# hobincar/reconstruction-network-for-video-captioning

Measured on AMD Instinct MI355X. Metric: captions/sec (train step) MSVD bs=100 28x1536 feats, higher is better.
Workload: dtype bf16; 1 GPU; decoder + global reconstructor train step (fwd+bwd+clip+Adam), B=100 per GPU, F=28, D=R=1536, V=4188, E=468, H=512, A=128, T=31, dropout 0.5, LSTM cells; global_batch=100, parallelism=dp1, hipgraph=True, deferred_reconstructor_update=True, grad_allreduce=False

## Files before the change

reconstruction-network-for-video-captioning_amd/csrc/abi_step.inc:

```

int recnet_set_deferred_reconstructor_update(recnet_handle* h, int32_t on, void* stream) {
  REQUIRE_WS(h);
  FLUSH_PENDING(h, stream);
  h->defer_rec = on ? (on == 2 ? 2 : 1) : 0;
  LAUNCH_OK();
  return RECNET_OK;
}
int recnet_flush(recnet_handle* h, void* stream) {
  REQUIRE_WS(h);
  int r = flush_pending(h, (hipStream_t)stream, 1); if (r) return r;
  LAUNCH_OK();
  return RECNET_OK;
}
int recnet_set_dp_overlap(recnet_handle* h, int32_t on) {
  if (!h) return fail(RECNET_EINVAL, "null handle");
  h->ss.dp_overlap = on ? 1 : 0;
  return RECNET_OK;
}
int recnet_join_side(recnet_handle* h, void* stream) {
  REQUIRE_WS(h);
  if (h->ss.side_open && h->s2) { hipEventRecord(h->ev[EV_REC_DW_JOIN], h->s2); hipStreamWaitEvent((hipStream_t)stream, h->ev[EV_REC_DW_JOIN], 0); }
  h->ss.side_open = 0;
  LAUNCH_OK();
  return RECNET_OK;
}
int recnet_abort_step(recnet_handle* h) {
  if (!h) return fail(RECNET_EINVAL, "null handle");
  sched_reset(h);
  return RECNET_OK;
}
int recnet_mark_pending(recnet_handle* h) {
  if (!h) return fail(RECNET_EINVAL, "null handle");
  if (h->defer_rec) { h->maybe_pending = 1; h->images_maybe_stale = 1; }
  return RECNET_OK;
}

int recnet_forward_decoder(recnet_handle* h, const float* enc, const int64_t* targets, int32_t T,
                           const float* step_weight, int32_t train, uint32_t seed, float* hiddens_out,
                           recnet_scalars* scalars, void* stream) {
  REQUIRE_WS(h);
  if (!h->dec_bound) return fail(RECNET_ESTATE, "decoder not bound");
  if (!enc || !targets || !step_weight) return fail(RECNET_EINVAL, "null argument");
  if (check_T(h, T)) return fail(RECNET_EINVAL, "T out of range");
  hipStream_t st = (hipStream_t)stream;
  hipLaunchKernelGGL(set_u32_kernel, dim3(1), dim3(1), 0, st, h->ctrl, seed);
  int r = fwd_decoder(h, enc, targets, T, step_weight, train, hiddens_out, st); if (r) return r;
  if (scalars) hipLaunchKernelGGL(export_scalars_kernel, dim3(1), dim3(1), 0, st, h->scal, scalars);
  LAUNCH_OK();
  return RECNET_OK;
}

int recnet_forward_decoder_free(recnet_handle* h, const float* enc, const int64_t* targets, int32_t T,
                                const float* step_weight, int32_t train, uint32_t seed, float* hiddens_out,
                                int64_t* output_indices, recnet_scalars* scalars, void* stream) {
  REQUIRE_WS(h);
  if (!h->dec_bound) return fail(RECNET_ESTATE, "decoder not bound");
// ... 29 lines not shown
  return RECNET_OK;
}

int recnet_backward_reconstructor(recnet_handle* h, const float* enc, float grad_scale, float* dhiddens_out, void* stream) {
  REQUIRE_WS(h);
  FLUSH_PENDING(h, stream);
  h->ss.prezeroed = 0;
  if (!h->fwd_rec_done) return fail(RECNET_ESTATE, "backward_reconstructor before forward_reconstructor");
  if (!h->rG.out_weight) return fail(RECNET_ESTATE, "reconstructor gradients not bound");
  hipStream_t st = (hipStream_t)stream;
  float* dh = dhiddens_out ? dhiddens_out : h->dHsrec;
  int r = bwd_rec(h, grad_scale, dh, st);
  if (r) return r;
  if (dhiddens_out) copyf(dhiddens_out, h->dHsrec, (size_t)h->T_last * h->B * h->H, st);
  h->rec_bwd_done = 1;
  (void)enc;
  LAUNCH_OK();
  return RECNET_OK;
}

int recnet_backward_decoder(recnet_handle* h, const float* enc, const int64_t* targets, const float* dhiddens,
                            float grad_scale, void* stream) {
  REQUIRE_WS(h);
  h->ss.prezeroed = 0;
  if (!h->fwd_dec_done) return fail(RECNET_ESTATE, "backward_decoder before forward_decoder");
  if (!h->dGd.out_weight) return fail(RECNET_ESTATE, "decoder gradients not bound");
  if (!enc || !targets) return fail(RECNET_EINVAL, "null argument");
  int r = bwd_decoder(h, enc, targets, dhiddens, grad_scale, (hipStream_t)stream); if (r) return r;
  h->fwd_dec_done = 0;
  LAUNCH_OK();
  return RECNET_OK;
}

int recnet_add_reg_grad(recnet_handle* h, int32_t which, float grad_scale, void* stream) {
  REQUIRE_WS(h);
  FLUSH_PENDING(h, stream);
  if (which < 0 || which > 1 || !h->og[which].bound) return fail(RECNET_EINVAL, "model not bound");
  OptGroup& o = h->og[which];
  const float lam = which == 0 ? h->c.decoder_lambda_reg : h->c.reconstructor_lambda_reg;
  hipLaunchKernelGGL(add_reg_grad_kernel, dim3(o.nchunks), dim3(256), 0, (hipStream_t)stream, o.d_tab, o.d_chunks, o.d_pnorm, lam * grad_scale);
  LAUNCH_OK();
  return RECNET_OK;
}

int recnet_clip_grad_norm(recnet_handle* h, int32_t which, float max_norm, float* total_norm_out, void* stream) {
  REQUIRE_WS(h);
// ... 50 lines not shown
  const bool rec = h->kind != RECNET_REC_NONE && !h->ss.defer_now;
  hipStream_t sd = h->s2;
  hipStream_t sn = h->ss.hoist_par ? sd : st;
  h->ss.hoist_pending = 0;
  if (sn != st) { if (h->ss.hoist_fork_recorded) hipStreamWaitEvent(sd, h->ev[EV_HOIST_FORK], 0); else fork_to(h, EV_HOIST_FORK, st, sd); }
  if (sn != st && h->persist_dec) wait_chain(h, 0, sn);
  param_norms(h, 0, h->scal + RN_SCAL_DEC_REG, sn);
  if (rec) { param_norms(h, 1, h->scal + RN_SCAL_REC_REG, sn); gate_bias(h->rP.rnn_bias_ih_l0, h->rP.rnn_bias_hh_l0, h->bsum_r, h->R, h->rgru, sn); }
  if (split_upd) gate_bias(h->rP.rnn_bias_ih_l0, h->rP.rnn_bias_hh_l0, h->bsum_r, h->R, h->rgru, sn);
  {
    ZeroList z; z.cnt = 0;
    auto add = [&](float* p, size_t n) { if (p && n) { z.p[z.cnt] = p; z.n[z.cnt] = n; ++z.cnt; } };
    add(h->dGd.embedding_weight, (size_t)h->V * h->E); add(h->dGd.out_bias, h->V); add(h->bsum4, (size_t)4 * h->H);
    add(h->dGd.attn_b, h->A); add(h->dGd.attn_w_weight, h->A);
    if (rec || split_upd) { add(h->rG.out_bias, h->R); add(h->bsum4r, (size_t)4 * h->R); }
    hipLaunchKernelGGL(zero_list_kernel, dim3(512), dim3(256), 0, sn, z);
    h->ss.prezeroed = 1;
  }
  if (h->kind == RECNET_REC_GLOBAL) {
    hipLaunchKernelGGL(mean_over_f_kernel, dim3(ew_blocks((size_t)h->B * h->D)), dim3(256), 0, sn, h->ss.hoist_enc, h->B, h->F, h->D, h->encmean);
    h->ss.encmean_hoisted = 1;
  }
  if (sn != st) hipEventRecord(h->ev[EV_HOIST_DONE], sd);
}

static void side_after_decoder_fwd(recnet_handle* h, hipStream_t st) {
  hipStream_t sd = h->overlap ? h->s2 : st;
  const bool par = sd != st;
  h->ss.side_pending = 0;
  if (par) {
    if (h->ss.side_fork_recorded) {
      hipStreamWaitEvent(sd, h->ev[EV_SIDE_FORK], 0);
      if (h->kind == RECNET_REC_GLOBAL && h->persist_rec) wait_chain(h, 2, sd);
    } else fork_to(h, EV_SIDE_FORK, st, sd);
    h->ss.side_fork_recorded = 0; h->ss.gws_cur = h->gws2;
  }
  h->ss.join_pending = par; h->ss.join_recorded = 0; h->ss.side_tail_open = 0;
  if (par && h->kind != RECNET_REC_NONE) h->ss.gg_slots = 2 * (h->ncu > 192 ? h->ncu - 192 : 32);
  int r = dec_fwd_loss(h, h->ss.side_targets, h->ss.side_T, h->ss.side_stepw, 1, sd);
  if (!r) r = dec_bwd_out(h, 1.0f, sd);
  h->ss.gg_slots = 0;
  if (!r && par && h->ss.side_phase != 2) { dec_ctx_rows(h, h->ss.side_enc, 0, h->ss.side_T, sd); h->ss.ctx_done = 1; }
  if (h->ss.side_tail_open) hipEventRecord(h->ev[EV_SIDE_TAIL], sd);
  h->ss.gws_cur = h->gws;
  h->ss.side_err = r;
}

static int fwd_bwd_impl(recnet_handle* h, const float* enc, const int64_t* targets, int T, const float* stepw, hipStream_t st,
                        int phase, int early_opt) {
  const bool rec = h->kind != RECNET_REC_NONE;
  hipStream_t sd = h->overlap ? h->s2 : st;
  const bool par = sd != st;
  int r;
  bool s3_join = false;
  const float* dh = rec ? h->dHsrec : nullptr;
  h->ss.early_opt_done = 0;
  if (phase != 2) h->free_fwd = 0;
  if (phase != 2) h->ss.ctx_done = 0;
  const bool defer_static = h->defer_rec && (h->kind == RECNET_REC_GLOBAL || (h->defer_rec == 2 && h->kind == RECNET_REC_LOCAL)) && phase == 0 && early_opt >= 0 && par && h->s3 &&
                            (h->defer_rec != 2 || h->split_ok);
  const bool defer = defer_static && (h->defer_rec != 2 || T >= 2);
  if (!defer && h->defer_rec && phase != 2) {
    if (defer_static) { const int fr = flush_pending(h, st, 1); if (fr) return fr; }
    else if (h->maybe_pending) { const int fr = flush_pending(h, st, 0); if (fr) return fr; }
  }
  h->ss.defer_now = defer ? 1 : 0;
  h->ss.img_defer_now = (!defer_static && h->defer_rec && rec && h->lp && phase == 0 && early_opt >= 0 && par && h->s3 &&
                      (h->persist_rec_bwd || h->persist_loc_bwd || h->persist_big_bwd || (h->persist_loc && h->lc_steps))) ? 1 : 0;
  if (defer) h->defer_flags = early_opt;
  if (phase != 2) {
    h->ss.hoist_pending = 1; h->ss.hoist_enc = enc; h->ss.hoist_par = par ? 1 : 0;
    h->ss.norms_hoisted = 1;
    r = dec_fwd_chain(h, enc, targets, T, 1, st);
    if (h->ss.hoist_pending) hoist_side_work(h, st);
    if (!r && h->ss.defer_err) { r = h->ss.defer_err; h->ss.defer_err = 0; }
    if (r) { h->ss.norms_hoisted = 0; return r; }
    h->ss.side_targets = targets; h->ss.side_stepw = stepw; h->ss.side_enc = enc; h->ss.side_T = T; h->ss.side_phase = phase; h->ss.side_err = 0;
    h->ss.side_pending = 1;
    if (!(par && h->kind == RECNET_REC_GLOBAL)) side_after_decoder_fwd(h, st);
// ... 52 lines not shown
    }
    h->ss.gws_cur = h->gws;
    if (r) { h->ss.defer_now = 0; return r; }
    if (h->kind == RECNET_REC_GLOBAL && T < h->Tm)
      hipMemsetAsync(at_off(h, h->dGr, (size_t)T * h->B * h->ld4R), 0, (size_t)(h->Tm - T) * h->B * h->ld4R * (h->lp ? 2 : 4), sd);
    hipLaunchKernelGGL(set_u32_kernel, dim3(1), dim3(1), 0, sd, h->ctrl + RN_CTRL_PENDING, 1u);
    h->maybe_pending = 1; h->ss.early_opt_done = 1; h->ss.deferred_done = 1;
  }
  if (phase == 0 && rec && !h->ss.deferred_done) {
    if (par) h->ss.gws_cur = h->gws2;
    if (par && h->persist_dec_bwd) wait_chain(h, 1, sd);
    r = bwd_rec_deferred(h, sd, 0); if (r) return r;
    h->ss.gws_cur = h->gws;
    if (early_opt >= 0 && par) {
      const int f_s3 = h->R >= 2560 ? 1 : 0;
      hipStream_t so = (f_s3 && h->s3) ? h->s3 : sd;
      if (so != sd) fork_to(h, EV_OPT_FORK, sd, so);
      r = optimizer_step(h, early_opt, so, 1); if (r) return r;
      h->ss.early_opt_done = 1;
      s3_join = so != sd;
    }
  }
  h->ss.deferred_done = 0;
  r = dec_bwd_chain(h, dh, st); if (r) return r;
  if (par) fork_to(h, EV_DEC_DW_FORK, st, sd);
  r = dec_bwd_deferred(h, enc, targets, st, par ? sd : nullptr, (par && h->s3 && !s3_join) ? h->s3 : nullptr);
  h->ss.ctx_done = 0;
  if (r) return r;
  if (par) join_from(h, EV_TAIL_JOIN, st, sd);
  if (s3_join) { if (h->ss.in_fused) h->ss.s3_late = 1; else join_from(h, EV_S3_JOIN, st, h->s3); }
  h->fwd_dec_done = 0;
  h->ss.prezeroed = 0;
  return RECNET_OK;
}

static int fwd_bwd(recnet_handle* h, const float* enc, const int64_t* targets, int T, const float* stepw, hipStream_t st,
                   int phase = 0, int early_opt = -1) {
  const int r = fwd_bwd_impl(h, enc, targets, T, stepw, st, phase, early_opt);
  if (!r && phase != 1 && early_opt < 0 && h->og[0].bound && h->og[0].tab[0].g)
    hipLaunchKernelGGL(poison_mark_kernel, dim3(1), dim3(1), 0, st, h->og[0].tab[0].g, (const float*)(h->scal + RN_SCAL_POISON));
  h->ss.defer_now = 0;
  if (r) sched_reset(h);
  return r;
}

static int check_step_args(recnet_handle* h, const float* enc, const int64_t* targets, int T, const float* step_weight) {
// ... 7 lines not shown
int recnet_train_step_fwd_bwd(recnet_handle* h, const float* enc, const int64_t* targets, int32_t T,
                              const float* step_weight, uint32_t seed, recnet_scalars* scalars, void* stream) {
  REQUIRE_WS(h);
  FLUSH_PENDING(h, stream);
  { const int cr = check_step_args(h, enc, targets, T, step_weight); if (cr) return cr; }
  hipStream_t st = (hipStream_t)stream;
  hipLaunchKernelGGL(set_u32_kernel, dim3(1), dim3(1), 0, st, h->ctrl, seed);
  int r = fwd_bwd(h, enc, targets, T, step_weight, st); if (r) return r;
  if (scalars) hipLaunchKernelGGL(export_scalars_kernel, dim3(1), dim3(1), 0, st, h->scal, scalars);
  h->fwd_dec_done = 0;
  LAUNCH_OK();
  return RECNET_OK;
}

static void step_fail_cleanup(recnet_handle* h, hipStream_t st) {
  if (h->ss.s3_late && h->s3) join_from(h, EV_S3_JOIN, st, h->s3);
  recnet_abort_step(h);
  if (h->defer_rec) { h->maybe_pending = 1; h->images_maybe_stale = 1; }
}

static int fused_step(recnet_handle* h, const float* enc, const int64_t* targets, int T, const float* step_weight, int flags,
                      recnet_scalars* scalars, hipStream_t st) {
  h->ss.in_fused = 1;
  int r = fwd_bwd(h, enc, targets, T, step_weight, st, 0, flags); if (r) { h->ss.in_fused = 0; return r; }
  r = optimizer_step(h, flags, st, h->ss.early_opt_done ? 0 : -1); h->ss.in_fused = 0;
  if (r) { step_fail_cleanup(h, st); return r; }
  if (h->ss.s3_late) { join_from(h, EV_S3_JOIN, st, h->s3); h->ss.s3_late = 0; }
  h->ss.img_defer_now = 0;
  if (scalars) hipLaunchKernelGGL(export_scalars_kernel, dim3(1), dim3(1), 0, st, h->scal, scalars);
  h->fwd_dec_done = 0;
  LAUNCH_OK();
  return RECNET_OK;
}

int recnet_train_step(recnet_handle* h, const float* enc, const int64_t* targets, int32_t T,
                      const float* step_weight, uint32_t seed, int32_t step, recnet_scalars* scalars, void* stream) {
  REQUIRE_WS(h);
  if (!h->defer_rec) { const int fr_ = flush_pending(h, (hipStream_t)stream); if (fr_) return fr_; }
  int r = check_step_args(h, enc, targets, T, step_weight); if (r) return r;
  if (step < 1) return fail(RECNET_EINVAL, "step must be >= 1");
  hipStream_t st = (hipStream_t)stream;
  hipLaunchKernelGGL(set_u32_kernel, dim3(1), dim3(1), 0, st, h->ctrl, seed);
  hipLaunchKernelGGL(set_step_kernel, dim3(1), dim3(1), 0, st, (int32_t*)(h->ctrl + RN_CTRL_STEP), step);
  return fused_step(h, enc, targets, T, step_weight, RECNET_OPT_REG | RECNET_OPT_CLIP, scalars, st);
}

int recnet_train_step_dev(recnet_handle* h, const float* enc, const int64_t* targets, int32_t T, const float* step_weight,
                          uint32_t seed_base, int32_t flags, recnet_scalars* scalars, void* stream) {
  REQUIRE_WS(h);
  if (!h->defer_rec) { const int fr_ = flush_pending(h, (hipStream_t)stream); if (fr_) return fr_; }
  int r = check_step_args(h, enc, targets, T, step_weight); if (r) return r;
  hipStream_t st = (hipStream_t)stream;
  hipLaunchKernelGGL(advance_step_kernel, dim3(1), dim3(1), 0, st, (int32_t*)(h->ctrl + RN_CTRL_STEP), h->ctrl, seed_base);
  return fused_step(h, enc, targets, T, step_weight, flags, scalars, st);
}

int recnet_set_step(recnet_handle* h, int32_t step, void* stream) {
  REQUIRE_WS(h);
  hipLaunchKernelGGL(set_u32_kernel, dim3(1), dim3(1), 0, (hipStream_t)stream, h->ctrl + RN_CTRL_STEP, (uint32_t)step);
  LAUNCH_OK();
  return RECNET_OK;
}

int recnet_train_step_fwd_bwd_dev(recnet_handle* h, const float* enc, const int64_t* targets, int32_t T,
                                  const float* step_weight, uint32_t seed_base, recnet_scalars* scalars, void* stream) {
  REQUIRE_WS(h);
  FLUSH_PENDING(h, stream);
  { const int cr = check_step_args(h, enc, targets, T, step_weight); if (cr) return cr; }
  hipStream_t st = (hipStream_t)stream;
  hipLaunchKernelGGL(advance_step_kernel, dim3(1), dim3(1), 0, st, (int32_t*)(h->ctrl + RN_CTRL_STEP), h->ctrl, seed_base);
  int r = fwd_bwd(h, enc, targets, T, step_weight, st); if (r) return r;
  if (scalars) hipLaunchKernelGGL(export_scalars_kernel, dim3(1), dim3(1), 0, st, h->scal, scalars);
  h->fwd_dec_done = 0;
// ... 32 lines not shown
```

reconstruction-network-for-video-captioning_amd/csrc/api.hip:

```cpp
#include <hip/hip_runtime.h>
#include <math.h>
#include <stdio.h>
#include <stdlib.h>
#include <ctype.h>
#include <string.h>
#include <algorithm>
#include <string>
#include <vector>

#include "../../include/recnet_hip.h"
#include "kernels.hpp"
#include "rec_chain.hpp"
#include "dec_chain.hpp"
#include "loc_chain.hpp"
#include "loc_big.hpp"
#include "step_sched.hpp"
#include "weight_images.hpp"

static thread_local std::string g_err;
static int fail(int code, const std::string& m) { g_err = m; return code; }
#define HIPCHK(x) do { hipError_t e_ = (x); if (e_ != hipSuccess) return fail(RECNET_EHIP, std::string(#x) + ": " + hipGetErrorString(e_)); } while (0)
#define LAUNCH_OK() do { hipError_t e_ = hipGetLastError(); if (e_ != hipSuccess) return fail(RECNET_EHIP, std::string(__func__) + ": " + hipGetErrorString(e_)); } while (0)

static inline int cdiv(long a, long b) { return (int)((a + b - 1) / b); }
// ... 39 lines not shown
  void* hm_pan = nullptr;
  void* hd_pan = nullptr; void* WoT = nullptr;
  float *lb_part = nullptr, *lb_dxm = nullptr, *lb_dbeta = nullptr; void* WstT = nullptr; int persist_big_bwd = 0, lb_steps = 0, lb_sr = 0, lb_ncb = 0;
  void* Wst = nullptr; int lc_steps = 0, lc_sr = 0;
  void *lc_panh = nullptr, *lc_panx = nullptr; _Float16* lc_pw = nullptr;
  void *lc_pang = nullptr, *lc_panw = nullptr; float* lc_dx = nullptr; void* WihhT = nullptr;
  int lcb_msx = 1, lcb_rbu = 4, lc_bwd_done = 0;
  int lcb_xs = 0;
  float mse_scale = 0.f; int mse_nb = 0;
  float dout_scale = 0.f;
  unsigned long long* lc_ts = nullptr;
  int lc_ms = 1, lc_rb = 4, lc_ng = 0, lc_nc = 0;
  void* dG_pan = nullptr;
  void* WhhT = nullptr;
  int persist_rec_bwd = 0;
  int persist_loc = 0, persist_loc_bwd = 0;
  int persist_dec = 0;
  float* dc_G1 = nullptr; void* dc_pan = nullptr;
  int persist_dec_bwd = 0;
  int bgrp_loc = 0;
  int bgrp = 0;
  int defer_rec = 0, maybe_pending = 0, def_rows = 0, defer_flags = 3; hipStream_t s3 = nullptr; float* gws3 = nullptr;
  int images_maybe_stale = 0;
  int split_ok = 0;
  int ncu = 0;
  float* dc_G2 = nullptr; void* dc_pan2 = nullptr;
  void *Xcat_g, *Hr_lp, *hrmean_lp, *dout_lp, *dGr, *Xcat_r, *dUd_lp, *dWhr, *dWhrs, *Wr4_w;
  void *Wih_f, *Whh_w, *Wor_w, *Ur_w, *Wr_w, *Wihh_w;
  int persist_rec = 0;
  float *sr_logits, *sr_scores, *sr_h[2], *sr_c[2], *sr_hn, *sr_cn, *sr_cum[2], *sr_vals;
  int64_t *sr_tok[2], *sr_hist[2]; int32_t *sr_eos[2], *sr_idx;
  int64_t* in_tok = nullptr;
  int free_fwd = 0;
  size_t gws_floats, slab_floats;
  float* gws2 = nullptr;
  unsigned* gcnt = nullptr;
  int gg_site = 0;
  struct RnSw { int wait_chain = 1, mse_epi = 1, adam_epi = 1, dec_lw = 1, dec_xcat = 1, rec_epi = 2, rec_wide = 1, persist_ms = 0, gemm_group = 1; } sw;
  hipStream_t s2 = nullptr; hipEvent_t ev[RN_EV_COUNT] = {}; int overlap = 1;
  StepSched ss;
  recnet_decoder_tensors dP{}, dGd{}, dM{}, dV{}, dVm{};
  recnet_reconstructor_tensors rP{}, rG{}, rM{}, rV{}, rVm{};
  bool dec_bound = false, rec_bound = false;
  OptGroup og[2];
  WImage wimg[WI_COUNT];
  int T_last = 0, train_last = 0, fwd_dec_done = 0, fwd_rec_done = 0, rec_bwd_done = 0;
  int prof_on = 0; std::vector<hipEvent_t> prof_ev; size_t prof_used = 0;
};
static void sched_reset(recnet_handle* h) { h->ss = StepSched{}; h->ss.gws_cur = h->gws; }

static void set_dims(recnet_handle* h) {
  h->ldD = pad8(h->D); h->ldE = pad8(h->E); h->ldH = pad8(h->H); h->ldV = pad8(h->V); h->ldA = pad8(h->A);
  h->ld4H = pad8(4 * h->H); h->ldWS = pad8(4 * h->H + RN_FCH * h->A); h->ldKW = pad8(4 * h->H + RN_FCH * h->A);
  h->ldR = pad8(h->R); h->ld4R = pad8(4 * h->R); h->ldRA = pad8(h->RA); h->ldHR = pad8(h->H + h->R);
  h->ldRA4 = pad8(RN_TCH * h->RA); h->ld2H = pad8(2 * h->H);
  if (h->kind != RECNET_REC_LOCAL) return;
  int steps = (h->R + 127) / 128; steps += steps & 1;
  h->lc_steps = steps > 16 ? (steps <= 28 ? 28 : 32) : 0; h->lc_sr = LC_HYB_SR(h->lc_steps);
  if (h->R > 2048 && h->R % 128 == 0 && h->B <= 64 * 2 * RN_MAX_ROW_GROUPS) {
    h->lb_steps = h->R / 128; h->lb_sr = LB_SR(h->lb_steps); h->lb_ncb = (h->H + h->R) / 64;
  }
// ... 222 lines not shown
int recnet_create(const recnet_config* cfg, recnet_handle** out) {
  if (!cfg || !out) return fail(RECNET_EINVAL, "null argument");
  const recnet_config& c = *cfg;
  if (c.batch_size <= 0 || c.encoder_output_len <= 0 || c.encoder_output_size <= 0 || c.embedding_size <= 0 ||
      c.decoder_hidden_size <= 0 || c.decoder_attn_size <= 0 || c.n_vocabs <= 3 || c.caption_max_len <= 0)
    return fail(RECNET_EINVAL, "non-positive dimension");
  if (c.reconstructor_type < 0 || c.reconstructor_type > 2) return fail(RECNET_EINVAL, "unknown reconstructor_type");
  if (c.precision != RECNET_PREC_F32 && c.precision != RECNET_PREC_BF16) return fail(RECNET_EINVAL, "unknown precision");
  if (c.decoder_attn_normalize != RECNET_ATTN_NONE && c.decoder_attn_normalize != RECNET_ATTN_SOFTMAX)
    return fail(RECNET_EINVAL, "unknown decoder_attn_normalize (0 = none, 1 = softmax)");
  if (c.decoder_cell < 0 || c.decoder_cell > 1 || c.reconstructor_cell < 0 || c.reconstructor_cell > 1)
    return fail(RECNET_EINVAL, "unknown recurrent cell (0 = LSTM, 1 = GRU)");
  if (c.reconstructor_type != RECNET_REC_NONE && c.reconstructor_hidden_size <= 0)
    return fail(RECNET_EINVAL, "reconstructor_hidden_size");
  if (c.reconstructor_type == RECNET_REC_LOCAL && c.reconstructor_hidden_size != c.encoder_output_size)
    return fail(RECNET_EINVAL, "local reconstructor requires reconstructor_hidden_size == encoder_output_size (train.py:128)");
  if (c.reconstructor_type == RECNET_REC_GLOBAL && c.reconstructor_hidden_size != c.encoder_output_size)
    return fail(RECNET_EINVAL, "global reconstructor requires reconstructor_hidden_size == encoder_output_size (train.py:101)");
  if (c.reconstructor_type == RECNET_REC_LOCAL && c.reconstructor_attn_size <= 0)
    return fail(RECNET_EINVAL, "reconstructor_attn_size");
  const std::vector<std::string> per_step = env_list("RN_PER_STEP"), alts = env_list("RN_ALT");
  const std::vector<std::string> per_step_names = {"dec", "dec_bwd", "rec", "rec_bwd", "loc", "loc_bwd", "loc_big", "all"};
  const std::vector<std::string> alt_names = {"dec_wh_in_phase_a", "dec_no_xcat", "rec_epilogue_0", "rec_epilogue_1", "rec_bwd_narrow",
                                              "rec_row_parts_1", "rec_row_parts_2", "loc_no_hybrid", "loc_xsplit_never", "loc_xsplit_always"};
  for (const std::string& t : per_step) if (!has(per_step_names, t)) return fail(RECNET_EINVAL, "RN_PER_STEP: unknown name '" + t + "'");
  for (const std::string& t : alts) if (!has(alt_names, t)) return fail(RECNET_EINVAL, "RN_ALT: unknown name '" + t + "'");
  auto alt = [&](const char* name) { return has(alts, name); };
  auto chain_on = [&](const char* name) { return !has(per_step, name) && !has(per_step, "all"); };
  recnet_handle* h = new recnet_handle();
  h->c = c;
  h->oh[0] = {c.decoder_learning_rate, c.decoder_weight_decay, c.adam_beta1, c.adam_beta2, c.adam_eps};
  h->oh[1] = {c.reconstructor_learning_rate, c.reconstructor_weight_decay, c.adam_beta1, c.adam_beta2, c.adam_eps};
  if (h->c.global_batch_size <= 0) h->c.global_batch_size = c.batch_size;
  h->B = c.batch_size; h->F = c.encoder_output_len; h->D = c.encoder_output_size; h->E = c.embedding_size;
  h->H = c.decoder_hidden_size; h->A = c.decoder_attn_size; h->V = c.n_vocabs;
  h->R = c.reconstructor_type ? c.reconstructor_hidden_size : 0;
  h->RA = c.reconstructor_type == RECNET_REC_LOCAL ? c.reconstructor_attn_size : 0;
  h->cml = c.caption_max_len; h->Tm = c.caption_max_len + 1;
  h->kind = c.reconstructor_type; h->prec = c.precision; h->lp = c.precision == RECNET_PREC_BF16;
  {
    auto env = [](const char* n, int dflt) { const char* e = getenv(n); return e ? atoi(e) : dflt; };
    h->sw.wait_chain = env("RN_WAIT_CHAIN", 1); h->sw.mse_epi = env("RN_MSE_EPILOGUE", 1); h->sw.adam_epi = env("RN_ADAM_EPILOGUE", 1);
    h->sw.gemm_group = env("RN_GEMM_GROUP", 1);
    h->sw.dec_lw = !alt("dec_wh_in_phase_a");
    h->sw.dec_xcat = !alt("dec_no_xcat"); h->sw.rec_epi = alt("rec_epilogue_0") ? 0 : (alt("rec_epilogue_1") ? 1 : 2); h->sw.rec_wide = !alt("rec_bwd_narrow");
    h->sw.persist_ms = alt("rec_row_parts_1") ? 1 : (alt("rec_row_parts_2") ? 2 : 0);
  }
  h->dgru = c.decoder_cell == RECNET_CELL_GRU; h->rgru = c.reconstructor_type != RECNET_REC_NONE && c.reconstructor_cell == RECNET_CELL_GRU;
  {
    const char* eg = getenv("RN_ROW_GROUPS");
    int ng = (h->B + RC_PAN_ROWS - 1) / RC_PAN_ROWS;
    if (eg && atoi(eg) == 0 && ng > 1) ng = 0;
    h->bgrp = ng >= 1 && ng <= RN_MAX_ROW_GROUPS ? (h->B + ng - 1) / ng : h->B;
  }
  const int Bg = h->bgrp;
  {
    int dev = 0, ncu = 0;
    hipGetDevice(&dev);
    hipDeviceGetAttribute(&ncu, hipDeviceAttributeMultiprocessorCount, dev);
    h->ncu = ncu;
    h->persist_rec = chain_on("rec") && h->lp && h->kind == RECNET_REC_GLOBAL && Bg <= RC_PAN_ROWS && h->Tm <= 60 &&
                     (h->R & 7) == 0 && h->R <= 2048 && h->R / 8 <= ncu;
    const int N = 4 * h->H + h->A, NA = N / 16;
    h->persist_dec = chain_on("dec") && h->lp && h->Tm <= 60 && (h->H & 7) == 0 && h->H <= 512 && h->F <= 32 + DC_XF && h->A <= 128 &&
                     (N & 15) == 0 && Bg <= RC_PAN_ROWS && (NA > Bg ? NA : Bg) + 1 <= ncu;
    h->persist_rec_bwd = chain_on("rec_bwd") && h->persist_rec && (h->R & 15) == 0;
  }
  h->bgrp_loc = h->bgrp;
  {
// ... 195 lines not shown
  const size_t NG = h->rgru ? 3 : 4;
  if (local) { n = {RA, RA * R, RA * H, RA, NG * R * H, NG * R * R, NG * R, NG * R, R * R, R}; }
  else { n = {NG * R * 2 * H, NG * R * R, NG * R, NG * R, R * R, R}; }
  auto G = rec_list(grad, local);
  if (G.empty()) G.assign(P.size(), nullptr);
  auto M = rec_list(exp_avg, local), Vv = rec_list(exp_avg_sq, local), Vm = rec_list(max_exp_avg_sq, local);
  if (!M.empty() && (any_null(M) || Vv.empty() || any_null(Vv))) return fail(RECNET_EINVAL, "Adam state pointer is null");
  if (h->c.reconstructor_use_amsgrad && !M.empty() && (Vm.empty() || any_null(Vm)))
    return fail(RECNET_EINVAL, "amsgrad needs max_exp_avg_sq");
  build_group(h->og[1], P, G, M, Vv, Vm, n);
  h->rec_bound = true;
  return upload_tables(h, 1);
}

}

#include "host_common.inc"
#include "host_decoder.inc"
#include "host_reconstructor.inc"

extern "C" {

static void refresh_images(recnet_handle* h, int group, hipStream_t st);
static int flush_pending(recnet_handle* h, hipStream_t st, int explicit_call = 0) {
  if (h->images_maybe_stale && h->rec_bound) { refresh_images(h, 1, st); h->images_maybe_stale = 0; }
  if (!h->maybe_pending && !(explicit_call && h->defer_rec)) return RECNET_OK;
  h->maybe_pending = 0;
  if (h->kind == RECNET_REC_NONE || !h->og[1].bound || !h->og[1].tab[0].m) return RECNET_OK;
  return rec_pending_update(h, st, 0, h->defer_flags);
}
#define FLUSH_PENDING(h, st) do { int fr_ = flush_pending(h, (hipStream_t)(st)); if (fr_) return fr_; } while (0)

int recnet_pack_weights(recnet_handle* h, void* stream) {
  REQUIRE_WS(h);
  FLUSH_PENDING(h, stream);
  int r = pack_weights(h, (hipStream_t)stream); if (r) return r;
  LAUNCH_OK();
  return RECNET_OK;
}

#include "abi_search.inc"
#include "abi_step.inc"
#include "abi_misc.inc"
```

reconstruction-network-for-video-captioning_amd/csrc/host_common.inc:

```
static bool prof_take(recnet_handle* h, hipStream_t st, hipEvent_t* e0, hipEvent_t* e1) {
  *e0 = *e1 = nullptr;
  hipStreamCaptureStatus cs = hipStreamCaptureStatusNone;
  if (hipStreamIsCapturing(st, &cs) != hipSuccess || cs != hipStreamCaptureStatusNone) return false;
  if (h->prof_used + 2 > h->prof_ev.size()) {
    hipEvent_t a = nullptr, b = nullptr; hipEventCreate(&a); hipEventCreate(&b);
    h->prof_ev.push_back(a); h->prof_ev.push_back(b);
  }
  *e0 = h->prof_ev[h->prof_used++]; *e1 = h->prof_ev[h->prof_used++];
  return true;
}
#define REQUIRE_WS(h) do { if (!(h) || !(h)->ws) return fail(RECNET_ESTATE, "workspace not bound"); } while (0)
#define LAUNCH_AT(h, kern, grid, block, smem, st, ...)                                          \
  do { if ((h)->lp) hipLaunchKernelGGL((kern<bf16_t>), grid, block, smem, st, __VA_ARGS__);     \
       else hipLaunchKernelGGL((kern<float>), grid, block, smem, st, __VA_ARGS__); } while (0)

static int check_T(const recnet_handle* h, int T) { return (T >= 1 && T <= h->Tm) ? 0 : 1; }
inline void* at_off(const recnet_handle* h, void* p, size_t elems) {
  return (char*)p + elems * (h->lp ? 2 : 4);
}

#include <dlfcn.h>
struct RnRange {
  typedef int (*push_t)(const char*);
  typedef int (*pop_t)();
// ... 171 lines not shown
  hipLaunchKernelGGL(wait_chain_kernel, dim3(1), dim3(64), 0, st, reinterpret_cast<const unsigned long long*>(h->ctrl + RN_CTRL_STAMP_START), stamps + 2 * k, 30000u);
}
static void hoist_side_work(recnet_handle* h, hipStream_t st);
static void side_after_decoder_fwd(recnet_handle* h, hipStream_t st);
static void refresh_image(recnet_handle* h, int id, hipStream_t st, int src_cols = 0) {
  const WImage& d = h->wimg[id];
  if (!d.live || !(h->*d.field)) return;
  const WImage& s = h->wimg[d.from];
  const bf16_t* src = (const bf16_t*)(h->*s.field);
  bf16_t* dst = (bf16_t*)(h->*d.field);
  const int cols = src_cols ? src_cols : s.cols;
  const dim3 grid((unsigned)cdiv((long)d.rows, 256));
  if (d.how == WI_TRANSPOSE)
    hipLaunchKernelGGL(transpose_at_kernel<bf16_t>, dim3(cdiv(cols, 32), cdiv(d.ld, 32)), dim3(256), 0, st, src, s.ld, (int)s.rows, cols, dst, d.ld);
  else if (d.how == WI_STREAM_FWD)
    hipLaunchKernelGGL(lc_pack_stream_kernel, grid, dim3(256), 0, st, src, s.ld, h->R, h->H, h->lc_steps, h->lc_sr, dst, d.rows);
  else if (d.how == WI_STREAM_BWD)
    hipLaunchKernelGGL(lcbig_pack_stream_kernel, grid, dim3(256), 0, st, src, s.ld, h->R, h->lb_ncb, h->lb_steps, h->lb_sr, dst, d.rows);
}
static void refresh_images(recnet_handle* h, int group, hipStream_t st) {
  for (int id = 0; id < WI_COUNT; ++id)
    if (h->wimg[id].how != WI_DIRECT && h->wimg[id].group == group) refresh_image(h, id, st);
}
static void rec_images_after_update(recnet_handle* h, hipStream_t st, bool whh_skipped = false) {
  if (h->ss.img_defer_now) { h->images_maybe_stale = 1; return; }
  if (!whh_skipped || h->persist_big_bwd) { refresh_images(h, 1, st); return; }
  if (h->kind == RECNET_REC_GLOBAL) { refresh_image(h, WI_WOT, st); return; }
  if (h->kind == RECNET_REC_LOCAL && h->persist_loc_bwd) refresh_image(h, WI_WIHHT, st, h->wimg[WI_WIHH_W].src[0].nc);
}

static int pack_weights(recnet_handle* h, hipStream_t st) {
  for (int g = 0; g < 2; ++g) {
    const OptGroup& o = h->og[g];
    if (!o.bound) continue;
    hipLaunchKernelGGL(pack_chunk_kernel, dim3(o.nchunks), dim3(256), 0, st, (const TensorDesc*)o.d_tab, (const int2*)o.d_chunks, (const PackDesc*)o.d_pack, h->lp);
    refresh_images(h, g, st);
  }
  return RECNET_OK;
}

static void launch_dec_cell(recnet_handle* h, const DecCellArgs& a, hipStream_t st) {
  if (h->lp && (h->H & 7) == 0 && h->F <= 32 && h->A <= 128 && (h->ld4H & 7) == 0) {
    const size_t smv = (size_t)(h->A + ((h->F + 3) & ~3) + 4 * 512 + 16) * 4;
    hipLaunchKernelGGL(dec_cell_vec_kernel<bf16_t>, dim3(h->B, cdiv(h->H, 512)), dim3(256), smv, st, a);
    return;
  }
// ... 22 lines not shown
```

reconstruction-network-for-video-captioning_amd/csrc/host_reconstructor.inc:

```
static void lstm_pw(recnet_handle* h, int Hd, int S, int slab_ld, const float* X, int x_ld, const float* b1, const float* b2,
                    const float* c_prev, float* h_out, void* h_lp, int hlp_ld, void* h_lp2, int hlp2_ld, float* c_out,
                    float* acts, hipStream_t st) {
  LstmPwArgs p;
  p.B = h->B; p.Hd = Hd; p.S = S; p.gru = h->rgru; p.slab = h->slab; p.slab_stride = (size_t)h->B * slab_ld; p.slab_ld = slab_ld;
  p.X = X; p.x_ld = x_ld; p.b1 = b1; p.b2 = b2; p.c_prev = c_prev; p.h_out = h_out; p.h_ld = Hd;
  p.h_lp = h_lp; p.hlp_ld = hlp_ld; p.hlp_pad_from = Hd; p.h_lp2 = h_lp2; p.hlp2_ld = hlp2_ld; p.c_out = c_out; p.acts = acts;
  auto al16 = [](const void* q) { return (((uintptr_t)q) & 15) == 0; };
  const bool vec = (Hd & 3) == 0 && (slab_ld & 3) == 0 && (x_ld & 3) == 0 && (hlp_ld & 3) == 0 && (hlp2_ld & 3) == 0 &&
                   al16(p.slab) && al16(X) && al16(b1) && al16(b2) && al16(c_prev) && al16(h_out) && al16(c_out) && al16(acts) &&
                   (((uintptr_t)h_lp) & 7) == 0 && (((uintptr_t)h_lp2) & 7) == 0;
  if (vec) LAUNCH_AT(h, lstm_pw_vec_kernel, dim3(cdiv((long)h->B * (Hd >> 2), 256)), dim3(256), 0, st, p);
  else LAUNCH_AT(h, lstm_pw_kernel, dim3(cdiv((long)h->B * Hd, 256)), dim3(256), 0, st, p);
}
static void mean_over_t(recnet_handle* h, const float* X, int T, int Cn, float scale, float* out, void* out_lp, int ld_lp, hipStream_t st) {
  const size_t n = (size_t)h->B * (out_lp ? ld_lp : Cn);
  if (h->lp) hipLaunchKernelGGL(mean_over_t_kernel<bf16_t>, dim3(ew_blocks(n)), dim3(256), 0, st, X, T, h->B, Cn, scale, out, (bf16_t*)out_lp, ld_lp);
  else hipLaunchKernelGGL(mean_over_t_kernel<float>, dim3(ew_blocks(n)), dim3(256), 0, st, X, T, h->B, Cn, scale, out, (float*)out_lp, ld_lp);
}

template <typename K, typename Args>
static void rc_launch(recnet_handle* h, int site, K kern, dim3 grid, size_t smem, hipStream_t st, const Args& a) {
  if (smem > 64 * 1024) hipFuncSetAttribute(reinterpret_cast<const void*>(kern), hipFuncAttributeMaxDynamicSharedMemorySize, (int)smem);
  hipEvent_t e1 = nullptr;
  if (h->prof_on == site) {
// ... 574 lines not shown
    }
    e.ad_pnorm = o.d_pnorm + ti;
  };
  if (!h->rgru) add(0, 4 * R, 0, dG1);
  else { add(0, 2 * R, 0, dG1); add((size_t)2 * R, R, (size_t)3 * R, at_off(h, (void*)dG1, (size_t)3 * R)); }
  h->gg_site = 3;
  if (!gg_run(h, g, s, &sh)) return false;
  if (local) { refresh_image(h, WI_WST, s); refresh_image(h, WI_WSTT, s); }
  return true;
}
static int optimizer_step(recnet_handle* h, int flags, hipStream_t st, int only_group, int deferred, int step_off, unsigned skip_mask) {
  RN_RANGE("recnet: norms + clip + Adam (train.py:270-273)");
  for (int g = 0; g < 2; ++g) {
    OptGroup& o = h->og[g];
    if (!o.bound) continue;
    if (only_group >= 0 && g != only_group) continue;
    if (g == 0 && (flags & RECNET_OPT_SKIP_DECODER)) continue;
    if (g == 1 && ((flags & RECNET_OPT_SKIP_RECONSTRUCTOR) || h->kind == RECNET_REC_NONE)) continue;
    if (!o.tab[0].m || !o.tab[0].g) return fail(RECNET_ESTATE, "gradients / Adam state not bound");
    AdamHyper hp = adam_hyper(h, g, flags);
    const float coef = hp.reg_coef;
    const float* clip = nullptr;
    if (g == 0 && (flags & RECNET_OPT_CLIP) && h->c.gradient_clip > 0.f) {
      hipLaunchKernelGGL(sumsq_chunk_kernel, dim3(o.nchunks), dim3(256), 0, st, o.d_tab, o.d_chunks, 1, o.d_pnorm, coef, o.d_partial);
      if (o.ntens <= 16) {
        hipLaunchKernelGGL(norm_all_kernel, dim3(1), dim3(256), 0, st, o.d_tab, o.d_partial, o.ntens, o.d_gnorm, h->c.gradient_clip, h->scal + RN_SCAL_GNORM, h->scal + RN_SCAL_CLIP, (float*)nullptr);
      } else {
        hipLaunchKernelGGL(tensor_norm_kernel, dim3(o.ntens), dim3(256), 0, st, o.d_tab, o.d_partial, o.d_gnorm);
        hipLaunchKernelGGL(norm_finalize_kernel, dim3(1), dim3(64), 0, st, o.d_gnorm, o.ntens, h->c.gradient_clip, h->scal + RN_SCAL_GNORM, h->scal + RN_SCAL_CLIP, (float*)nullptr);
      }
      clip = h->scal + RN_SCAL_CLIP;
    }
    hipLaunchKernelGGL(adam_chunk_kernel, dim3(o.nchunks), dim3(256), 0, st, o.d_tab, o.d_chunks, hp, o.d_pnorm, clip,
                       (const int32_t*)(h->ctrl + RN_CTRL_STEP), (const PackDesc*)o.d_pack, h->lp, (const float*)(h->scal + RN_SCAL_POISON),
                       deferred ? (const uint32_t*)(h->ctrl + RN_CTRL_PENDING) : (const uint32_t*)nullptr, step_off, g == 1 ? skip_mask : 0u);
    if (g == 0) refresh_images(h, 0, st);
    if (g == 1) rec_images_after_update(h, st, (skip_mask >> RN_REC_T_WHH(h)) & 1u);
  }
  return RECNET_OK;
}
```

reconstruction-network-for-video-captioning_amd/csrc/step_sched.hpp:

```cpp
#pragma once
#include <stdint.h>

enum RnEvent {
  EV_SIDE_FORK = 0, EV_SIDE_JOIN = 1, EV_BPTT_FORK = 2, EV_TAIL_JOIN = 3, EV_HOIST_FORK = 4, EV_HOIST_DONE = 5, EV_DEC_DW_FORK = 6,
  EV_XE_FORK = 8, EV_XE_JOIN = 9, EV_REC_DW_FORK = 10, EV_S3_FORK = 11, EV_S3_JOIN = 11, EV_PENDING_DONE = 12, EV_OPT_FORK = 13,
  EV_REC_DW_JOIN = 14, EV_TAIL2_FORK = 15, EV_TAIL3_FORK = 16, EV_TAIL3_JOIN = 17, EV_SIDE_TAIL = 18, EV_WHH_NORM = 21,
  RN_EV_COUNT = 24
};

struct StepSched {
  int side_pending = 0, side_T = 0, side_phase = 0, side_err = 0;
  const int64_t* side_targets = nullptr; const float* side_stepw = nullptr; const float* side_enc = nullptr;
  int hoist_pending = 0, hoist_par = 0; const float* hoist_enc = nullptr;
  int hoist_fork_recorded = 0;
  int side_fork_recorded = 0;
  int norms_hoisted = 0;
  int encmean_hoisted = 0;
  int join_pending = 0;
  int join_recorded = 0;
  int side_tail_open = 0;
  int total_late = 0;
  int rec_loss_defer = 0;
  int rec_loss_late = 0;
  int rec_norm_late = 0;
  int rec_wait_pending = 0;
  int deferred_early = 0, deferred_early_flags = -1, deferred_done = 0;
  int defer_now = 0;
  int defer_err = 0;
  int img_defer_now = 0;
  int s3_late = 0;
  int in_fused = 0;
  int gg_slots = 0;
  int gemm_single_group = 0;
  float* gws_cur = nullptr;

  int dp_overlap = 0;
  int side_open = 0;
  int prezeroed = 0;
  int xcat_done = 0;
  int mp_done = 0;
  int dhr_done = 0;
  int dout_ready = 0;
  int early_opt_done = 0;
  int ctx_done = 0;
};
```

Measured before the change: 68530 captions/s.

## Defer decoder weight-image refresh and compute tail grad norms early on side stream

Two tail-of-step changes. After the decoder Adam update in the fused step, the refresh of the derived decoder weight images is no longer done inline; it is marked stale and redone lazily in the next step's hoisted side work (or before an explicit backward). Separately, the sum-of-squares for the last decoder gradient tensors, which are final before the decoder backward chain, is launched on the side stream so it overlaps that chain, and the optimizer's norm pass only covers the remaining chunks. Both aim to shorten the serial critical path at the step tail, at the cost of more stale-state bookkeeping and a hard-coded ntens==11 assumption.

```diff
diff --git a/reconstruction-network-for-video-captioning_amd/csrc/abi_step.inc b/reconstruction-network-for-video-captioning_amd/csrc/abi_step.inc
--- a/reconstruction-network-for-video-captioning_amd/csrc/abi_step.inc
+++ b/reconstruction-network-for-video-captioning_amd/csrc/abi_step.inc
@@ -32,6 +32,7 @@
 int recnet_mark_pending(recnet_handle* h) {
   if (!h) return fail(RECNET_EINVAL, "null handle");
   if (h->defer_rec) { h->maybe_pending = 1; h->images_maybe_stale = 1; }
+  if (dec_images_lazy_ok(h)) h->dec_images_stale = 1;
   return RECNET_OK;
 }
 
@@ -107,6 +108,7 @@
 int recnet_backward_decoder(recnet_handle* h, const float* enc, const int64_t* targets, const float* dhiddens,
                             float grad_scale, void* stream) {
   REQUIRE_WS(h);
+  if (h->dec_images_stale) { refresh_images(h, 0, (hipStream_t)stream); h->dec_images_stale = 0; }
   h->ss.prezeroed = 0;
   if (!h->fwd_dec_done) return fail(RECNET_ESTATE, "backward_decoder before forward_decoder");
   if (!h->dGd.out_weight) return fail(RECNET_ESTATE, "decoder gradients not bound");
@@ -203,6 +205,7 @@
     h->ss.encmean_hoisted = 1;
   }
   if (sn != st) hipEventRecord(h->ev[EV_HOIST_DONE], sd);
+  if (h->ss.in_fused && dec_images_lazy_ok(h)) { refresh_images(h, 0, sn); h->dec_images_stale = 0; }
 }
 
 static void side_after_decoder_fwd(recnet_handle* h, hipStream_t st) {
@@ -236,6 +239,13 @@
   bool s3_join = false;
   const float* dh = rec ? h->dHsrec : nullptr;
   h->ss.early_opt_done = 0;
+  {
+    const OptGroup& o = h->og[0];
+    h->ss.norm_early_done = 0;
+    h->ss.norm_early = (h->ss.in_fused && h->sw.tail_fast && h->lp && h->sw.gemm_group && phase == 0 && early_opt >= 0 && (early_opt & RECNET_OPT_CLIP) &&
+                        !(early_opt & RECNET_OPT_SKIP_DECODER) && h->c.gradient_clip > 0.f && o.bound && o.ntens == 11 && o.tab[0].g && o.tab[0].m) ? 1 : 0;
+    h->ss.norm_early_coef = h->ss.norm_early ? adam_hyper(h, 0, early_opt).reg_coef : 0.f;
+  }
   if (phase != 2) h->free_fwd = 0;
   if (phase != 2) h->ss.ctx_done = 0;
   const bool defer_static = h->defer_rec && (h->kind == RECNET_REC_GLOBAL || (h->defer_rec == 2 && h->kind == RECNET_REC_LOCAL)) && phase == 0 && early_opt >= 0 && par && h->s3 &&
@@ -334,6 +344,12 @@
     }
   }
   h->ss.deferred_done = 0;
+  if (h->ss.norm_early && par) {
+    OptGroup& o = h->og[0];
+    const int c0 = o.tab[o.ntens - 2].chunk0;
+    hipLaunchKernelGGL(sumsq_chunk_kernel, dim3(o.nchunks - c0), dim3(256), 0, sd, o.d_tab, o.d_chunks + c0, 1, o.d_pnorm, h->ss.norm_early_coef, o.d_partial + c0);
+    h->ss.norm_early_done = c0;
+  }
   r = dec_bwd_chain(h, dh, st); if (r) return r;
   if (par) fork_to(h, EV_DEC_DW_FORK, st, sd);
   r = dec_bwd_deferred(h, enc, targets, st, par ? sd : nullptr, (par && h->s3 && !s3_join) ? h->s3 : nullptr);
@@ -387,7 +403,7 @@
 static int fused_step(recnet_handle* h, const float* enc, const int64_t* targets, int T, const float* step_weight, int flags,
                       recnet_scalars* scalars, hipStream_t st) {
   h->ss.in_fused = 1;
-  int r = fwd_bwd(h, enc, targets, T, step_weight, st, 0, flags); if (r) { h->ss.in_fused = 0; return r; }
+  int r = fwd_bwd(h, enc, targets, T, step_weight, st, 0, flags); h->ss.norm_early = 0; if (r) { h->ss.in_fused = 0; return r; }
   r = optimizer_step(h, flags, st, h->ss.early_opt_done ? 0 : -1); h->ss.in_fused = 0;
   if (r) { step_fail_cleanup(h, st); return r; }
   if (h->ss.s3_late) { join_from(h, EV_S3_JOIN, st, h->s3); h->ss.s3_late = 0; }
@@ -401,7 +417,7 @@
 int recnet_train_step(recnet_handle* h, const float* enc, const int64_t* targets, int32_t T,
                       const float* step_weight, uint32_t seed, int32_t step, recnet_scalars* scalars, void* stream) {
   REQUIRE_WS(h);
-  if (!h->defer_rec) { const int fr_ = flush_pending(h, (hipStream_t)stream); if (fr_) return fr_; }
+  if (!h->defer_rec) { const int fr_ = flush_pending(h, (hipStream_t)stream, 0, dec_images_lazy_ok(h)); if (fr_) return fr_; }
   int r = check_step_args(h, enc, targets, T, step_weight); if (r) return r;
   if (step < 1) return fail(RECNET_EINVAL, "step must be >= 1");
   hipStream_t st = (hipStream_t)stream;
@@ -413,7 +429,7 @@
 int recnet_train_step_dev(recnet_handle* h, const float* enc, const int64_t* targets, int32_t T, const float* step_weight,
                           uint32_t seed_base, int32_t flags, recnet_scalars* scalars, void* stream) {
   REQUIRE_WS(h);
-  if (!h->defer_rec) { const int fr_ = flush_pending(h, (hipStream_t)stream); if (fr_) return fr_; }
+  if (!h->defer_rec) { const int fr_ = flush_pending(h, (hipStream_t)stream, 0, dec_images_lazy_ok(h)); if (fr_) return fr_; }
   int r = check_step_args(h, enc, targets, T, step_weight); if (r) return r;
   hipStream_t st = (hipStream_t)stream;
   hipLaunchKernelGGL(advance_step_kernel, dim3(1), dim3(1), 0, st, (int32_t*)(h->ctrl + RN_CTRL_STEP), h->ctrl, seed_base);
diff --git a/reconstruction-network-for-video-captioning_amd/csrc/api.hip b/reconstruction-network-for-video-captioning_amd/csrc/api.hip
--- a/reconstruction-network-for-video-captioning_amd/csrc/api.hip
+++ b/reconstruction-network-for-video-captioning_amd/csrc/api.hip
@@ -85,6 +85,7 @@
   int bgrp = 0;
   int defer_rec = 0, maybe_pending = 0, def_rows = 0, defer_flags = 3; hipStream_t s3 = nullptr; float* gws3 = nullptr;
   int images_maybe_stale = 0;
+  int dec_images_stale = 0;
   int split_ok = 0;
   int ncu = 0;
   float* dc_G2 = nullptr; void* dc_pan2 = nullptr;
@@ -99,7 +100,7 @@
   float* gws2 = nullptr;
   unsigned* gcnt = nullptr;
   int gg_site = 0;
-  struct RnSw { int wait_chain = 1, mse_epi = 1, adam_epi = 1, dec_lw = 1, dec_xcat = 1, rec_epi = 2, rec_wide = 1, persist_ms = 0, gemm_group = 1; } sw;
+  struct RnSw { int wait_chain = 1, mse_epi = 1, adam_epi = 1, dec_lw = 1, dec_xcat = 1, rec_epi = 2, rec_wide = 1, persist_ms = 0, gemm_group = 1, tail_fast = 1; } sw;
   hipStream_t s2 = nullptr; hipEvent_t ev[RN_EV_COUNT] = {}; int overlap = 1;
   StepSched ss;
   recnet_decoder_tensors dP{}, dGd{}, dM{}, dV{}, dVm{};
@@ -368,7 +369,7 @@
   const std::vector<std::string> per_step = env_list("RN_PER_STEP"), alts = env_list("RN_ALT");
   const std::vector<std::string> per_step_names = {"dec", "dec_bwd", "rec", "rec_bwd", "loc", "loc_bwd", "loc_big", "all"};
   const std::vector<std::string> alt_names = {"dec_wh_in_phase_a", "dec_no_xcat", "rec_epilogue_0", "rec_epilogue_1", "rec_bwd_narrow",
-                                              "rec_row_parts_1", "rec_row_parts_2", "loc_no_hybrid", "loc_xsplit_never", "loc_xsplit_always"};
+                                              "rec_row_parts_1", "rec_row_parts_2", "loc_no_hybrid", "loc_xsplit_never", "loc_xsplit_always", "tail_norm_pass"};
   for (const std::string& t : per_step) if (!has(per_step_names, t)) return fail(RECNET_EINVAL, "RN_PER_STEP: unknown name '" + t + "'");
   for (const std::string& t : alts) if (!has(alt_names, t)) return fail(RECNET_EINVAL, "RN_ALT: unknown name '" + t + "'");
   auto alt = [&](const char* name) { return has(alts, name); };
@@ -391,6 +392,7 @@
     h->sw.dec_lw = !alt("dec_wh_in_phase_a");
     h->sw.dec_xcat = !alt("dec_no_xcat"); h->sw.rec_epi = alt("rec_epilogue_0") ? 0 : (alt("rec_epilogue_1") ? 1 : 2); h->sw.rec_wide = !alt("rec_bwd_narrow");
     h->sw.persist_ms = alt("rec_row_parts_1") ? 1 : (alt("rec_row_parts_2") ? 2 : 0);
+    h->sw.tail_fast = !alt("tail_norm_pass");
   }
   h->dgru = c.decoder_cell == RECNET_CELL_GRU; h->rgru = c.reconstructor_type != RECNET_REC_NONE && c.reconstructor_cell == RECNET_CELL_GRU;
   {
@@ -632,8 +634,9 @@
 extern "C" {
 
 static void refresh_images(recnet_handle* h, int group, hipStream_t st);
-static int flush_pending(recnet_handle* h, hipStream_t st, int explicit_call = 0) {
+static int flush_pending(recnet_handle* h, hipStream_t st, int explicit_call = 0, int keep_dec = 0) {
   if (h->images_maybe_stale && h->rec_bound) { refresh_images(h, 1, st); h->images_maybe_stale = 0; }
+  if (h->dec_images_stale && h->dec_bound && !keep_dec) { refresh_images(h, 0, st); h->dec_images_stale = 0; }
   if (!h->maybe_pending && !(explicit_call && h->defer_rec)) return RECNET_OK;
   h->maybe_pending = 0;
   if (h->kind == RECNET_REC_NONE || !h->og[1].bound || !h->og[1].tab[0].m) return RECNET_OK;
diff --git a/reconstruction-network-for-video-captioning_amd/csrc/host_common.inc b/reconstruction-network-for-video-captioning_amd/csrc/host_common.inc
--- a/reconstruction-network-for-video-captioning_amd/csrc/host_common.inc
+++ b/reconstruction-network-for-video-captioning_amd/csrc/host_common.inc
@@ -217,6 +217,7 @@
   for (int id = 0; id < WI_COUNT; ++id)
     if (h->wimg[id].how != WI_DIRECT && h->wimg[id].group == group) refresh_image(h, id, st);
 }
+static bool dec_images_lazy_ok(const recnet_handle* h) { return h->sw.tail_fast && h->wimg[WI_WCOMBT].live && h->WcombT; }
 static void rec_images_after_update(recnet_handle* h, hipStream_t st, bool whh_skipped = false) {
   if (h->ss.img_defer_now) { h->images_maybe_stale = 1; return; }
   if (!whh_skipped || h->persist_big_bwd) { refresh_images(h, 1, st); return; }
diff --git a/reconstruction-network-for-video-captioning_amd/csrc/host_reconstructor.inc b/reconstruction-network-for-video-captioning_amd/csrc/host_reconstructor.inc
--- a/reconstruction-network-for-video-captioning_amd/csrc/host_reconstructor.inc
+++ b/reconstruction-network-for-video-captioning_amd/csrc/host_reconstructor.inc
@@ -620,7 +620,9 @@
     const float coef = hp.reg_coef;
     const float* clip = nullptr;
     if (g == 0 && (flags & RECNET_OPT_CLIP) && h->c.gradient_clip > 0.f) {
-      hipLaunchKernelGGL(sumsq_chunk_kernel, dim3(o.nchunks), dim3(256), 0, st, o.d_tab, o.d_chunks, 1, o.d_pnorm, coef, o.d_partial);
+      const int nch = h->ss.norm_early_done ? h->ss.norm_early_done : o.nchunks;
+      h->ss.norm_early_done = 0;
+      hipLaunchKernelGGL(sumsq_chunk_kernel, dim3(nch), dim3(256), 0, st, o.d_tab, o.d_chunks, 1, o.d_pnorm, coef, o.d_partial);
       if (o.ntens <= 16) {
         hipLaunchKernelGGL(norm_all_kernel, dim3(1), dim3(256), 0, st, o.d_tab, o.d_partial, o.ntens, o.d_gnorm, h->c.gradient_clip, h->scal + RN_SCAL_GNORM, h->scal + RN_SCAL_CLIP, (float*)nullptr);
       } else {
@@ -632,7 +634,7 @@
     hipLaunchKernelGGL(adam_chunk_kernel, dim3(o.nchunks), dim3(256), 0, st, o.d_tab, o.d_chunks, hp, o.d_pnorm, clip,
                        (const int32_t*)(h->ctrl + RN_CTRL_STEP), (const PackDesc*)o.d_pack, h->lp, (const float*)(h->scal + RN_SCAL_POISON),
                        deferred ? (const uint32_t*)(h->ctrl + RN_CTRL_PENDING) : (const uint32_t*)nullptr, step_off, g == 1 ? skip_mask : 0u);
-    if (g == 0) refresh_images(h, 0, st);
+    if (g == 0) { if (h->ss.in_fused && dec_images_lazy_ok(h)) h->dec_images_stale = 1; else refresh_images(h, 0, st); }
     if (g == 1) rec_images_after_update(h, st, (skip_mask >> RN_REC_T_WHH(h)) & 1u);
   }
   return RECNET_OK;
diff --git a/reconstruction-network-for-video-captioning_amd/csrc/step_sched.hpp b/reconstruction-network-for-video-captioning_amd/csrc/step_sched.hpp
--- a/reconstruction-network-for-video-captioning_amd/csrc/step_sched.hpp
+++ b/reconstruction-network-for-video-captioning_amd/csrc/step_sched.hpp
@@ -42,5 +42,6 @@
   int dhr_done = 0;
   int dout_ready = 0;
   int early_opt_done = 0;
+  int norm_early = 0, norm_early_done = 0; float norm_early_coef = 0.f;
   int ctx_done = 0;
 };
```

Result: no change. 68880 captions/s (median of 6 runs) (+0.5%).
